# edouardoyallon/acco

Hardware: NVIDIA H100
Metric: tokens/sec (device-timed, max over ranks) Llama ACCO bf16 sharded-Adam, 8x1024 tokens per GPU per micro-batch (higher is better)
Workload: dtype bf16

## Files before the change

acco_b200/csrc/attention_wgmma.cu:

```cuda
#include <cuda.h>
#include <cuda_bf16.h>
#include <cuda_runtime.h>
#include <math.h>
#include <stdint.h>

#include "wgmma.cuh"

namespace acco_attn {

using namespace acco_tc;

constexpr int HD = 64;
constexpr int LDS = HD + 8;
constexpr float LOG2E = 1.4426950408889634f;
constexpr float LN2 = 0.6931471805599453f;

typedef __nv_bfloat16 bf16;

__device__ __forceinline__ uint32_t pack2(float a, float b) {
    __nv_bfloat162 h = __floats2bfloat162_rn(a, b);
    return *reinterpret_cast<uint32_t*>(&h);
}
__device__ __forceinline__ uint32_t ld32(const bf16* p) { return *reinterpret_cast<const uint32_t*>(p); }

__device__ __forceinline__ void mma16816(float (&c)[4], const uint32_t (&a)[4], uint32_t b0, uint32_t b1) {
    asm volatile("mma.sync.aligned.m16n8k16.row.col.f32.bf16.bf16.f32 {%0,%1,%2,%3}, {%4,%5,%6,%7}, {%8,%9}, {%0,%1,%2,%3};"
                 : "+f"(c[0]), "+f"(c[1]), "+f"(c[2]), "+f"(c[3])
                 : "r"(a[0]), "r"(a[1]), "r"(a[2]), "r"(a[3]), "r"(b0), "r"(b1));
}

template <int NB, int KB>
__device__ __forceinline__ void warp_mma_ss(float (&acc)[NB][4], const bf16* A, const bf16* B, int lane) {
    const int g = lane >> 2, t = lane & 3;
#pragma unroll
    for (int kb = 0; kb < KB; ++kb) {
        uint32_t a[4];
        const bf16* a0 = A + g * LDS + kb * 16 + 2 * t;
        a[0] = ld32(a0); a[1] = ld32(a0 + 8 * LDS); a[2] = ld32(a0 + 8); a[3] = ld32(a0 + 8 * LDS + 8);
#pragma unroll
        for (int nb = 0; nb < NB; ++nb) {
            const bf16* b = B + (nb * 8 + g) * LDS + kb * 16 + 2 * t;
            mma16816(acc[nb], a, ld32(b), ld32(b + 8));
        }
    }
}
template <int NB>
__device__ __forceinline__ void warp_mma_rs(float (&acc)[NB][4], const float (&p)[8][4], const bf16* B, int lane) {
    const int g = lane >> 2, t = lane & 3;
#pragma unroll
    for (int kb = 0; kb < 4; ++kb) {
        uint32_t a[4];
        a[0] = pack2(p[2 * kb][0], p[2 * kb][1]);
        a[1] = pack2(p[2 * kb][2], p[2 * kb][3]);
        a[2] = pack2(p[2 * kb + 1][0], p[2 * kb + 1][1]);
        a[3] = pack2(p[2 * kb + 1][2], p[2 * kb + 1][3]);
#pragma unroll
        for (int nb = 0; nb < NB; ++nb) {
            const bf16* b = B + (nb * 8 + g) * LDS + kb * 16 + 2 * t;
            mma16816(acc[nb], a, ld32(b), ld32(b + 8));
        }
    }
}

__device__ __forceinline__ void load_tile(bf16* dst, const bf16* src, long long ld, int rows, int valid, int tid, int nthr) {
    for (int i = tid; i < rows * 8; i += nthr) {
        const int r = i >> 3, c = (i & 7) * 8;
        uint4 v = make_uint4(0, 0, 0, 0);
        if (r < valid) v = *reinterpret_cast<const uint4*>(src + (long long)r * ld + c);
        *reinterpret_cast<uint4*>(dst + r * LDS + c) = v;
    }
}
__device__ __forceinline__ void load_tile_t(bf16* dst, const bf16* src, long long ld, int rows, int tid, int nthr) {
    for (int i = tid; i < rows * 8; i += nthr) {
        const int r = i >> 3, c = (i & 7) * 8;
        const uint4 v = *reinterpret_cast<const uint4*>(src + (long long)r * ld + c);
        const bf16* e = reinterpret_cast<const bf16*>(&v);
#pragma unroll
        for (int j = 0; j < 8; ++j) dst[(c + j) * LDS + r] = e[j];
    }
}

__device__ __forceinline__ bool visible(int q, int kv, int window) { return kv <= q && kv > q - window; }

struct FwdParams {
    CUtensorMap map_q;
    CUtensorMap map_k;
    CUtensorMap map_v;
    bf16* o;
    long long ld_o;
    float* lse;
    int B, S, Hq, Hk, window;
    float scale;
    const int* seg;
};

constexpr int FWD_Q = 128, FWD_KV = 64, FWD_THREADS = 256;
constexpr int FWD_TILE_KV = FWD_KV * HD * 2;
constexpr int FWD_SMEM = FWD_Q * HD * 2 + 2 * 2 * FWD_TILE_KV + 1024  + 64 ;

__device__ __forceinline__ void wgmma_m64n64k16_rs_tb(float (&d)[32], const uint32_t (&a)[4], uint64_t db) {
    asm volatile(
        "{\n\t.reg .pred p;\n\tsetp.ne.b32 p, %37, 0;\n\twgmma.mma_async.sync.aligned.m64n64k16.f32.bf16.bf16 "
        "{%0,%1,%2,%3,%4,%5,%6,%7,%8,%9,%10,%11,%12,%13,%14,%15,%16,%17,%18,%19,%20,%21,%22,%23,%24,%25,%26,%27,%28,%29,%30,%31}, "
        "{%32,%33,%34,%35}, %36, p, 1, 1, 1;\n\t}"
        : "+f"(d[0]), "+f"(d[1]), "+f"(d[2]), "+f"(d[3]), "+f"(d[4]), "+f"(d[5]), "+f"(d[6]), "+f"(d[7]), "+f"(d[8]), "+f"(d[9]), "+f"(d[10]),
          "+f"(d[11]), "+f"(d[12]), "+f"(d[13]), "+f"(d[14]), "+f"(d[15]), "+f"(d[16]), "+f"(d[17]), "+f"(d[18]), "+f"(d[19]), "+f"(d[20]),
          "+f"(d[21]), "+f"(d[22]), "+f"(d[23]), "+f"(d[24]), "+f"(d[25]), "+f"(d[26]), "+f"(d[27]), "+f"(d[28]), "+f"(d[29]), "+f"(d[30]),
          "+f"(d[31])
        : "r"(a[0]), "r"(a[1]), "r"(a[2]), "r"(a[3]), "l"(db), "r"(1));
}

template <bool kSeg>
__global__ void __launch_bounds__(FWD_THREADS) attn_fwd_kernel(const __grid_constant__ FwdParams P) {
    extern __shared__ uint8_t smem_raw[];
    uint8_t* smem = (uint8_t*)(((uintptr_t)smem_raw + 1023) & ~(uintptr_t)1023);
    uint8_t* sQ = smem;
    uint8_t* sKV = smem + FWD_Q * HD * 2;
    uint64_t* full = (uint64_t*)(sKV + 2 * 2 * FWD_TILE_KV);
    const int qb = blockIdx.x, h = blockIdx.y, b = blockIdx.z;
    const int hk = h / (P.Hq / P.Hk);
    const int tid = threadIdx.x, wg = tid >> 7, warp = (tid >> 5) & 3, lane = tid & 31, g = lane >> 2, t = lane & 3;
    const int q0 = qb * FWD_Q;
    const int row0 = b * P.S;
    int lo_key = max(0, q0 - P.window + 1);
    if constexpr (kSeg) lo_key = max(lo_key, P.seg[row0 + q0]);
    const int j_lo = lo_key / FWD_KV, j_hi = (q0 + FWD_Q - 1) / FWD_KV;
    auto issue = [&](int j) {
        const int s = (j - j_lo) & 1;
        mbar_expect_tx(&full[s], 2 * FWD_TILE_KV);
        tma_load_2d(&P.map_k, &full[s], sKV + s * 2 * FWD_TILE_KV, hk * HD, row0 + j * FWD_KV);
        tma_load_2d(&P.map_v, &full[s], sKV + s * 2 * FWD_TILE_KV + FWD_TILE_KV, hk * HD, row0 + j * FWD_KV);
    };
    if (tid == 0) {
        mbar_init(&full[0], 1);
        mbar_init(&full[1], 1);
        mbar_init(&full[2], 1);
        asm volatile("fence.mbarrier_init.release.cluster;" ::: "memory");
        mbar_expect_tx(&full[2], FWD_Q * HD * 2);
        tma_load_2d(&P.map_q, &full[2], sQ, h * HD, row0 + q0);
        issue(j_lo);
        if (j_lo + 1 <= j_hi) issue(j_lo + 1);
    }
    __syncthreads();
    mbar_wait(&full[2], 0);
    const float c = P.scale * LOG2E;
    float m_run[2] = {-INFINITY, -INFINITY}, l_run[2] = {0.f, 0.f};
    float o[32];
#pragma unroll
    for (int i = 0; i < 32; ++i) o[i] = 0.f;
    const int wq_lo = q0 + wg * 64, wq_hi = wq_lo + 63;
    const int qr[2] = {wq_lo + warp * 16 + g, wq_lo + warp * 16 + g + 8};
    int sg[2] = {0, 0}, wseg = 0;
    if constexpr (kSeg) {
        sg[0] = P.seg[row0 + qr[0]];
        sg[1] = P.seg[row0 + qr[1]];
        wseg = P.seg[row0 + wq_lo];
    }
    const uint32_t q_addr = smem_u32(sQ) + (uint32_t)(wg * 8192);
    for (int j = j_lo; j <= j_hi; ++j) {
        const int kv0 = j * FWD_KV, s = (j - j_lo) & 1;
        mbar_wait(&full[s], (uint32_t)(((j - j_lo) >> 1) & 1));
        if (!(kv0 > wq_hi || kv0 + FWD_KV - 1 <= wq_lo - P.window || (kSeg && kv0 + FWD_KV - 1 < wseg))) {
            const uint32_t k_addr = smem_u32(sKV + s * 2 * FWD_TILE_KV), v_addr = k_addr + FWD_TILE_KV;
            float sc[32];
#pragma unroll
            for (int i = 0; i < 32; ++i) sc[i] = 0.f;
            wgmma_fence();
#pragma unroll
            for (int k = 0; k < HD / 16; ++k)
                wgmma_m64n64k16<0, 0>(sc, make_smem_desc(q_addr + k * 32, 1, 1024 >> 4), make_smem_desc(k_addr + k * 32, 1, 1024 >> 4), 1u);
            wgmma_commit();
            wgmma_wait<0>();
            reg_fence(sc);
            float mx[2] = {-INFINITY, -INFINITY};
#pragma unroll
            for (int nb = 0; nb < 8; ++nb)
#pragma unroll
                for (int e = 0; e < 4; ++e) {
                    const int kv = kv0 + nb * 8 + 2 * t + (e & 1), r = e >> 1;
                    const float v = visible(qr[r], kv, P.window) && (!kSeg || kv >= sg[r]) ? sc[4 * nb + e] * c : -INFINITY;
                    sc[4 * nb + e] = v;
                    mx[r] = fmaxf(mx[r], v);
                }
#pragma unroll
            for (int r = 0; r < 2; ++r) {
                mx[r] = fmaxf(mx[r], __shfl_xor_sync(0xffffffffu, mx[r], 1));
                mx[r] = fmaxf(mx[r], __shfl_xor_sync(0xffffffffu, mx[r], 2));
            }
            float alpha[2], base[2], rs[2] = {0.f, 0.f};
#pragma unroll
            for (int r = 0; r < 2; ++r) {
                const float m_new = fmaxf(m_run[r], mx[r]);
                base[r] = m_new == -INFINITY ? 0.f : m_new;
                alpha[r] = exp2f(m_run[r] - base[r]);
                m_run[r] = m_new;
            }
#pragma unroll
            for (int i = 0; i < 32; ++i) {
                const int r = (i >> 1) & 1;
                const float p = exp2f(sc[i] - base[r]);
                sc[i] = p;
                rs[r] += p;
            }
#pragma unroll
            for (int r = 0; r < 2; ++r) {
                rs[r] += __shfl_xor_sync(0xffffffffu, rs[r], 1);
                rs[r] += __shfl_xor_sync(0xffffffffu, rs[r], 2);
                l_run[r] = l_run[r] * alpha[r] + rs[r];
            }
#pragma unroll
            for (int i = 0; i < 32; ++i) o[i] *= alpha[(i >> 1) & 1];
            wgmma_fence();
#pragma unroll
            for (int kk = 0; kk < FWD_KV / 16; ++kk) {
                uint32_t a[4];
                a[0] = pack2(sc[8 * kk + 0], sc[8 * kk + 1]);
                a[1] = pack2(sc[8 * kk + 2], sc[8 * kk + 3]);
                a[2] = pack2(sc[8 * kk + 4], sc[8 * kk + 5]);
                a[3] = pack2(sc[8 * kk + 6], sc[8 * kk + 7]);
                wgmma_m64n64k16_rs_tb(o, a, make_smem_desc(v_addr + kk * 2048, 8192 >> 4, 1024 >> 4));
            }
            wgmma_commit();
            wgmma_wait<0>();
            reg_fence(o);
        }
        __syncthreads();
        if (tid == 0 && j + 2 <= j_hi) issue(j + 2);
    }
#pragma unroll
    for (int r = 0; r < 2; ++r) {
        const int q = qr[r];
        const float inv = l_run[r] > 0.f ? 1.f / l_run[r] : 0.f;
        bf16* dst = P.o + ((long long)row0 + q) * P.ld_o + h * HD + 2 * t;
#pragma unroll
        for (int nb = 0; nb < 8; ++nb)
            *reinterpret_cast<uint32_t*>(dst + nb * 8) = pack2(o[4 * nb + 2 * r] * inv, o[4 * nb + 2 * r + 1] * inv);
        if (t == 0) P.lse[((long long)b * P.Hq + h) * P.S + q] = (m_run[r] + log2f(l_run[r])) * LN2;
    }
}

struct BwdParams {
    const bf16 *q, *k, *v;
    long long ld;
    const bf16* d_o;
    long long ld_do;
    const float *lse, *delta;
    float* dq;
    bf16 *dk, *dv;
    int B, S, Hq, Hk, window;
    float scale;
    const int* seg;
};

constexpr int BWD_KV = 64, BWD_Q = 64, BWD_THREADS = 128;
constexpr int BWD_SMEM = 8 * 64 * LDS * 2 + 2 * BWD_Q * 4;
constexpr int BWD_SMEM_SEG = BWD_SMEM + (BWD_Q + 1) * 4;

template <bool kSeg>
__global__ void __launch_bounds__(BWD_THREADS) attn_bwd_kernel(const BwdParams P) {
    extern __shared__ __align__(16) uint8_t smem_raw[];
    bf16* sK = reinterpret_cast<bf16*>(smem_raw);
    bf16* sKt = sK + 64 * LDS;
    bf16* sV = sKt + 64 * LDS;
    bf16* sQ = sV + 64 * LDS;
    bf16* sQt = sQ + 64 * LDS;
    bf16* sdO = sQt + 64 * LDS;
    bf16* sdOt = sdO + 64 * LDS;
    bf16* sdS = sdOt + 64 * LDS;
    float* sL = reinterpret_cast<float*>(sdS + 64 * LDS);
    float* sD = sL + BWD_Q;
    int* sSeg = reinterpret_cast<int*>(sD + BWD_Q);
    const int nb_k = blockIdx.x, hk = blockIdx.y, b = blockIdx.z;
    const int G = P.Hq / P.Hk;
    const int tid = threadIdx.x, warp = tid >> 5, lane = tid & 31, g = lane >> 2, t = lane & 3;
    const int kv0 = nb_k * BWD_KV;
    const long long row0 = (long long)b * P.S;
    load_tile(sK, P.k + (row0 + kv0) * P.ld + hk * HD, P.ld, BWD_KV, BWD_KV, tid, BWD_THREADS);
    load_tile_t(sKt, P.k + (row0 + kv0) * P.ld + hk * HD, P.ld, BWD_KV, tid, BWD_THREADS);
    load_tile(sV, P.v + (row0 + kv0) * P.ld + hk * HD, P.ld, BWD_KV, BWD_KV, tid, BWD_THREADS);
    const float c = P.scale * LOG2E;
    float dk[8][4], dv[8][4];
#pragma unroll
    for (int i = 0; i < 8; ++i)
#pragma unroll
        for (int e = 0; e < 4; ++e) dk[i][e] = dv[i][e] = 0.f;
    const int kr[2] = {kv0 + warp * 16 + g, kv0 + warp * 16 + g + 8};
    const int m_lo = kv0 / BWD_Q;
    const int m_hi = min(P.S / BWD_Q - 1, (kv0 + BWD_KV - 1 + P.window - 1) / BWD_Q);
    for (int gi = 0; gi < G; ++gi) {
        const int hq = hk * G + gi;
        for (int m = m_lo; m <= m_hi; ++m) {
            const int q0 = m * BWD_Q;
            __syncthreads();
            load_tile(sQ, P.q + (row0 + q0) * P.ld + hq * HD, P.ld, BWD_Q, BWD_Q, tid, BWD_THREADS);
            load_tile_t(sQt, P.q + (row0 + q0) * P.ld + hq * HD, P.ld, BWD_Q, tid, BWD_THREADS);
            load_tile(sdO, P.d_o + (row0 + q0) * P.ld_do + hq * HD, P.ld_do, BWD_Q, BWD_Q, tid, BWD_THREADS);
            load_tile_t(sdOt, P.d_o + (row0 + q0) * P.ld_do + hq * HD, P.ld_do, BWD_Q, tid, BWD_THREADS);
            if (tid < BWD_Q) {
                const long long li = ((long long)b * P.Hq + hq) * P.S + q0 + tid;
                sL[tid] = P.lse[li] * LOG2E;
                sD[tid] = P.delta[li];
                if constexpr (kSeg) sSeg[tid] = P.seg[row0 + q0 + tid];
            }
            if (kSeg && tid == BWD_Q) sSeg[BWD_Q] = m == m_hi || P.seg[row0 + q0 + BWD_Q] > kv0 + BWD_KV - 1;
            __syncthreads();
            float s[8][4], dp[8][4];
#pragma unroll
            for (int i = 0; i < 8; ++i)
#pragma unroll
                for (int e = 0; e < 4; ++e) s[i][e] = dp[i][e] = 0.f;
            warp_mma_ss<8, 4>(s, sK + warp * 16 * LDS, sQ, lane);
            warp_mma_ss<8, 4>(dp, sV + warp * 16 * LDS, sdO, lane);
#pragma unroll
            for (int nb = 0; nb < 8; ++nb)
#pragma unroll
                for (int e = 0; e < 4; ++e) {
                    const int ql = nb * 8 + 2 * t + (e & 1), q = q0 + ql, r = e >> 1;
                    const float p = visible(q, kr[r], P.window) && (!kSeg || kr[r] >= sSeg[ql]) ? exp2f(s[nb][e] * c - sL[ql]) : 0.f;
                    const float pb = __bfloat162float(__float2bfloat16(p));
                    s[nb][e] = pb;
                    dp[nb][e] = __bfloat162float(__float2bfloat16(p * (dp[nb][e] - sD[ql]) * P.scale));
                }
#pragma unroll
            for (int nb = 0; nb < 8; ++nb)
#pragma unroll
                for (int e = 0; e < 4; ++e) {
                    const int ql = nb * 8 + 2 * t + (e & 1), kl = warp * 16 + g + 8 * (e >> 1);
                    sdS[ql * LDS + kl] = __float2bfloat16(dp[nb][e]);
                }
            warp_mma_rs<8>(dv, s, sdOt, lane);
            warp_mma_rs<8>(dk, dp, sQt, lane);
            __syncthreads();
            float dq[8][4];
#pragma unroll
            for (int i = 0; i < 8; ++i) dq[i][0] = dq[i][1] = dq[i][2] = dq[i][3] = 0.f;
            warp_mma_ss<8, 4>(dq, sdS + warp * 16 * LDS, sKt, lane);
#pragma unroll
            for (int r = 0; r < 2; ++r) {
                float* dst = P.dq + (row0 + q0 + warp * 16 + g + 8 * r) * (long long)(P.Hq * HD) + hq * HD + 2 * t;
#pragma unroll
                for (int nb = 0; nb < 8; ++nb) {
                    atomicAdd(dst + nb * 8, dq[nb][2 * r]);
                    atomicAdd(dst + nb * 8 + 1, dq[nb][2 * r + 1]);
                }
            }
            if (kSeg && sSeg[BWD_Q]) break;
        }
    }
#pragma unroll
    for (int r = 0; r < 2; ++r) {
        const long long off = (row0 + kr[r]) * (long long)(P.Hk * HD) + hk * HD + 2 * t;
#pragma unroll
        for (int nb = 0; nb < 8; ++nb) {
            *reinterpret_cast<uint32_t*>(P.dk + off + nb * 8) = pack2(dk[nb][2 * r], dk[nb][2 * r + 1]);
            *reinterpret_cast<uint32_t*>(P.dv + off + nb * 8) = pack2(dv[nb][2 * r], dv[nb][2 * r + 1]);
        }
    }
}

__global__ void __launch_bounds__(256) attn_delta_kernel(const bf16* __restrict__ o, const bf16* __restrict__ d_o, long long ld_o,
                                                         long long ld_do, float* __restrict__ delta, int B, int S, int Hq) {
    const long long item = ((long long)blockIdx.x * blockDim.x + threadIdx.x) >> 3;
    const int part = threadIdx.x & 7;
    const long long n_items = (long long)B * S * Hq;
    float acc = 0.f;
    long long row = 0;
    int h = 0;
    if (item < n_items) {
        row = item / Hq;
        h = (int)(item - row * Hq);
        const uint4 a = *reinterpret_cast<const uint4*>(o + row * ld_o + h * HD + part * 8);
        const uint4 d = *reinterpret_cast<const uint4*>(d_o + row * ld_do + h * HD + part * 8);
        const __nv_bfloat162* a2 = reinterpret_cast<const __nv_bfloat162*>(&a);
        const __nv_bfloat162* d2 = reinterpret_cast<const __nv_bfloat162*>(&d);
#pragma unroll
        for (int i = 0; i < 4; ++i) {
            const float2 x = __bfloat1622float2(a2[i]), y = __bfloat1622float2(d2[i]);
            acc += x.x * y.x + x.y * y.y;
        }
    }
    acc += __shfl_xor_sync(0xffffffffu, acc, 1);
    acc += __shfl_xor_sync(0xffffffffu, acc, 2);
    acc += __shfl_xor_sync(0xffffffffu, acc, 4);
    if (item < n_items && part == 0) {
        const long long b = row / S, s = row - b * S;
        delta[(b * Hq + h) * S + s] = acc;
    }
}

static bool shape_ok(int B, int S, int Hq, int Hk, int D, float scale) {
    return B > 0 && S > 0 && S % 128 == 0 && Hk > 0 && Hq > 0 && Hq % Hk == 0 && D == HD && scale > 0.f;
}
static bool aligned(const void* p, long long ld) { return ((uintptr_t)p % 16) == 0 && (ld % 8) == 0; }
static int eff_window(int S, int window) { return (window <= 0 || window > S) ? S : window; }

}

extern "C" int acco_attn_supported(int B, int S, int Hq, int Hk, int D, float scale) {
    return acco_attn::shape_ok(B, S, Hq, Hk, D, scale) ? 1 : 0;
}

extern "C" int acco_attn_fwd(const void* q, const void* k, const void* v, long long ld, void* o, long long ld_o, float* lse, int B, int S, int Hq,
                             int Hk, int D, float scale, int window, const int* seg, cudaStream_t st) {
    using namespace acco_attn;
    if (!shape_ok(B, S, Hq, Hk, D, scale) || !aligned(q, ld) || !aligned(k, ld) || !aligned(v, ld) || !aligned(o, ld_o)) return -1;
    static int fwd_attr = (int)cudaFuncSetAttribute(attn_fwd_kernel<false>, cudaFuncAttributeMaxDynamicSharedMemorySize, FWD_SMEM);
    static int fwd_attr_seg = (int)cudaFuncSetAttribute(attn_fwd_kernel<true>, cudaFuncAttributeMaxDynamicSharedMemorySize, FWD_SMEM);
    if (fwd_attr) return fwd_attr;
    if (fwd_attr_seg) return fwd_attr_seg;
    FwdParams P;
    const uint64_t rows = (uint64_t)B * S;
    int rc = acco_gemm::make_map_typed(&P.map_q, q, (uint64_t)Hq * HD, rows, (uint64_t)ld, HD, FWD_Q, 2);
    if (!rc) rc = acco_gemm::make_map_typed(&P.map_k, k, (uint64_t)Hk * HD, rows, (uint64_t)ld, HD, FWD_KV, 2);
    if (!rc) rc = acco_gemm::make_map_typed(&P.map_v, v, (uint64_t)Hk * HD, rows, (uint64_t)ld, HD, FWD_KV, 2);
    if (rc) return rc;
    P.o = (bf16*)o; P.ld_o = ld_o; P.lse = lse;
    P.B = B; P.S = S; P.Hq = Hq; P.Hk = Hk; P.window = eff_window(S, window); P.scale = scale; P.seg = seg;
    if (seg)
        attn_fwd_kernel<true><<<dim3(S / FWD_Q, Hq, B), FWD_THREADS, FWD_SMEM, st>>>(P);
    else
        attn_fwd_kernel<false><<<dim3(S / FWD_Q, Hq, B), FWD_THREADS, FWD_SMEM, st>>>(P);
    return (int)cudaGetLastError();
}

extern "C" int acco_attn_bwd(const void* q, const void* k, const void* v, long long ld, const void* o, long long ld_o, const void* d_o,
                             long long ld_do, const float* lse, float* delta, float* dq_acc, void* dk, void* dv, int B, int S, int Hq, int Hk, int D,
                             float scale, int window, const int* seg, cudaStream_t st) {
    using namespace acco_attn;
    if (!shape_ok(B, S, Hq, Hk, D, scale) || !aligned(q, ld) || !aligned(k, ld) || !aligned(v, ld) || !aligned(o, ld_o) || !aligned(d_o, ld_do))
        return -1;
    static int attr_rc = (int)cudaFuncSetAttribute(attn_bwd_kernel<false>, cudaFuncAttributeMaxDynamicSharedMemorySize, BWD_SMEM);
    static int attr_rc_seg = (int)cudaFuncSetAttribute(attn_bwd_kernel<true>, cudaFuncAttributeMaxDynamicSharedMemorySize, BWD_SMEM_SEG);
    if (attr_rc) return attr_rc;
    if (attr_rc_seg) return attr_rc_seg;
    const long long items = (long long)B * S * Hq;
    attn_delta_kernel<<<(unsigned)((items * 8 + 255) / 256), 256, 0, st>>>((const bf16*)o, (const bf16*)d_o, ld_o, ld_do, delta, B, S, Hq);
    if (cudaMemsetAsync(dq_acc, 0, (size_t)items * HD * sizeof(float), st) != cudaSuccess) return -6;
    BwdParams P{(const bf16*)q, (const bf16*)k, (const bf16*)v, ld, (const bf16*)d_o, ld_do, lse, delta, dq_acc, (bf16*)dk, (bf16*)dv,
                B, S, Hq, Hk, eff_window(S, window), scale, seg};
    if (seg)
        attn_bwd_kernel<true><<<dim3(S / BWD_KV, Hk, B), BWD_THREADS, BWD_SMEM_SEG, st>>>(P);
    else
        attn_bwd_kernel<false><<<dim3(S / BWD_KV, Hk, B), BWD_THREADS, BWD_SMEM, st>>>(P);
    return (int)cudaGetLastError();
}
```

Measured before the change: 387,100.

## Rewrite attention backward with WGMMA, TMA double-buffering and TMA reduce for dQ

The attention backward kernel moves from warp-level mma.sync with manually transposed shared-memory tiles to Hopper WGMMA. It now uses two warpgroups over a 128-key block, TMA loads of Q/dO/LSE/delta double-buffered with mbarriers, and TMA reduce-add of dQ through a swizzled shared buffer in place of per-element atomics. This is meant to remove the scalar transpose loads, the redundant smem copies and the heavy global atomic traffic. The forward grid is reordered so heads come first and query blocks run in reverse order, putting the long causal blocks early. The cost is a large, complex kernel with new alignment requirements on lse/delta/seg and one block per SM.

```diff
diff --git a/acco_b200/csrc/attention_wgmma.cu b/acco_b200/csrc/attention_wgmma.cu
--- a/acco_b200/csrc/attention_wgmma.cu
+++ b/acco_b200/csrc/attention_wgmma.cu
@@ -11,7 +11,6 @@
 using namespace acco_tc;
 
 constexpr int HD = 64;
-constexpr int LDS = HD + 8;
 constexpr float LOG2E = 1.4426950408889634f;
 constexpr float LN2 = 0.6931471805599453f;
 
@@ -20,64 +19,6 @@
 __device__ __forceinline__ uint32_t pack2(float a, float b) {
     __nv_bfloat162 h = __floats2bfloat162_rn(a, b);
     return *reinterpret_cast<uint32_t*>(&h);
-}
-__device__ __forceinline__ uint32_t ld32(const bf16* p) { return *reinterpret_cast<const uint32_t*>(p); }
-
-__device__ __forceinline__ void mma16816(float (&c)[4], const uint32_t (&a)[4], uint32_t b0, uint32_t b1) {
-    asm volatile("mma.sync.aligned.m16n8k16.row.col.f32.bf16.bf16.f32 {%0,%1,%2,%3}, {%4,%5,%6,%7}, {%8,%9}, {%0,%1,%2,%3};"
-                 : "+f"(c[0]), "+f"(c[1]), "+f"(c[2]), "+f"(c[3])
-                 : "r"(a[0]), "r"(a[1]), "r"(a[2]), "r"(a[3]), "r"(b0), "r"(b1));
-}
-
-template <int NB, int KB>
-__device__ __forceinline__ void warp_mma_ss(float (&acc)[NB][4], const bf16* A, const bf16* B, int lane) {
-    const int g = lane >> 2, t = lane & 3;
-#pragma unroll
-    for (int kb = 0; kb < KB; ++kb) {
-        uint32_t a[4];
-        const bf16* a0 = A + g * LDS + kb * 16 + 2 * t;
-        a[0] = ld32(a0); a[1] = ld32(a0 + 8 * LDS); a[2] = ld32(a0 + 8); a[3] = ld32(a0 + 8 * LDS + 8);
-#pragma unroll
-        for (int nb = 0; nb < NB; ++nb) {
-            const bf16* b = B + (nb * 8 + g) * LDS + kb * 16 + 2 * t;
-            mma16816(acc[nb], a, ld32(b), ld32(b + 8));
-        }
-    }
-}
-template <int NB>
-__device__ __forceinline__ void warp_mma_rs(float (&acc)[NB][4], const float (&p)[8][4], const bf16* B, int lane) {
-    const int g = lane >> 2, t = lane & 3;
-#pragma unroll
-    for (int kb = 0; kb < 4; ++kb) {
-        uint32_t a[4];
-        a[0] = pack2(p[2 * kb][0], p[2 * kb][1]);
-        a[1] = pack2(p[2 * kb][2], p[2 * kb][3]);
-        a[2] = pack2(p[2 * kb + 1][0], p[2 * kb + 1][1]);
-        a[3] = pack2(p[2 * kb + 1][2], p[2 * kb + 1][3]);
-#pragma unroll
-        for (int nb = 0; nb < NB; ++nb) {
-            const bf16* b = B + (nb * 8 + g) * LDS + kb * 16 + 2 * t;
-            mma16816(acc[nb], a, ld32(b), ld32(b + 8));
-        }
-    }
-}
-
-__device__ __forceinline__ void load_tile(bf16* dst, const bf16* src, long long ld, int rows, int valid, int tid, int nthr) {
-    for (int i = tid; i < rows * 8; i += nthr) {
-        const int r = i >> 3, c = (i & 7) * 8;
-        uint4 v = make_uint4(0, 0, 0, 0);
-        if (r < valid) v = *reinterpret_cast<const uint4*>(src + (long long)r * ld + c);
-        *reinterpret_cast<uint4*>(dst + r * LDS + c) = v;
-    }
-}
-__device__ __forceinline__ void load_tile_t(bf16* dst, const bf16* src, long long ld, int rows, int tid, int nthr) {
-    for (int i = tid; i < rows * 8; i += nthr) {
-        const int r = i >> 3, c = (i & 7) * 8;
-        const uint4 v = *reinterpret_cast<const uint4*>(src + (long long)r * ld + c);
-        const bf16* e = reinterpret_cast<const bf16*>(&v);
-#pragma unroll
-        for (int j = 0; j < 8; ++j) dst[(c + j) * LDS + r] = e[j];
-    }
 }
 
 __device__ __forceinline__ bool visible(int q, int kv, int window) { return kv <= q && kv > q - window; }
@@ -117,9 +58,10 @@
     uint8_t* sQ = smem;
     uint8_t* sKV = smem + FWD_Q * HD * 2;
     uint64_t* full = (uint64_t*)(sKV + 2 * 2 * FWD_TILE_KV);
-    const int qb = blockIdx.x, h = blockIdx.y, b = blockIdx.z;
+    const int h = blockIdx.x, b = blockIdx.y, qb = gridDim.z - 1 - blockIdx.z;
     const int hk = h / (P.Hq / P.Hk);
-    const int tid = threadIdx.x, wg = tid >> 7, warp = (tid >> 5) & 3, lane = tid & 31, g = lane >> 2, t = lane & 3;
+    const int tid = threadIdx.x, warp = (tid >> 5) & 3, lane = tid & 31, g = lane >> 2, t = lane & 3;
+    const int wg = __shfl_sync(0xffffffffu, tid >> 7, 0);
     const int q0 = qb * FWD_Q;
     const int row0 = b * P.S;
     int lo_key = max(0, q0 - P.window + 1);
@@ -240,120 +182,188 @@
 }
 
 struct BwdParams {
-    const bf16 *q, *k, *v;
-    long long ld;
-    const bf16* d_o;
-    long long ld_do;
+    CUtensorMap map_q;
+    CUtensorMap map_k;
+    CUtensorMap map_v;
+    CUtensorMap map_do;
+    CUtensorMap map_dq;
     const float *lse, *delta;
-    float* dq;
     bf16 *dk, *dv;
     int B, S, Hq, Hk, window;
     float scale;
     const int* seg;
 };
 
-constexpr int BWD_KV = 64, BWD_Q = 64, BWD_THREADS = 128;
-constexpr int BWD_SMEM = 8 * 64 * LDS * 2 + 2 * BWD_Q * 4;
-constexpr int BWD_SMEM_SEG = BWD_SMEM + (BWD_Q + 1) * 4;
+constexpr int BWD_KV = 128, BWD_Q = 64, BWD_THREADS = 256;
+constexpr int BWD_TILE = BWD_Q * HD * 2;
+constexpr int BWD_STAGE = 2 * BWD_TILE + 3 * BWD_Q * 4;
+constexpr int BWD_DQ = BWD_Q * HD * 4;
+constexpr int BWD_SMEM = 2 * 2 * BWD_TILE + 2 * BWD_TILE + 2 * BWD_DQ + 2 * BWD_STAGE + 1024  + 64 ;
+
+__device__ __forceinline__ void bulk_load(void* dst, const void* src, uint32_t bytes, uint64_t* bar) {
+    asm volatile("cp.async.bulk.shared::cluster.global.mbarrier::complete_tx::bytes [%0], [%1], %2, [%3];" ::"r"(smem_u32(dst)), "l"(src),
+                 "r"(bytes), "r"(smem_u32(bar))
+                 : "memory");
+}
 
 template <bool kSeg>
-__global__ void __launch_bounds__(BWD_THREADS) attn_bwd_kernel(const BwdParams P) {
-    extern __shared__ __align__(16) uint8_t smem_raw[];
-    bf16* sK = reinterpret_cast<bf16*>(smem_raw);
-    bf16* sKt = sK + 64 * LDS;
-    bf16* sV = sKt + 64 * LDS;
-    bf16* sQ = sV + 64 * LDS;
-    bf16* sQt = sQ + 64 * LDS;
-    bf16* sdO = sQt + 64 * LDS;
-    bf16* sdOt = sdO + 64 * LDS;
-    bf16* sdS = sdOt + 64 * LDS;
-    float* sL = reinterpret_cast<float*>(sdS + 64 * LDS);
-    float* sD = sL + BWD_Q;
-    int* sSeg = reinterpret_cast<int*>(sD + BWD_Q);
-    const int nb_k = blockIdx.x, hk = blockIdx.y, b = blockIdx.z;
+__global__ void __launch_bounds__(BWD_THREADS, 1) attn_bwd_kernel(const __grid_constant__ BwdParams P) {
+    extern __shared__ uint8_t smem_raw[];
+    uint8_t* smem = (uint8_t*)(((uintptr_t)smem_raw + 1023) & ~(uintptr_t)1023);
+    uint8_t* sK = smem;
+    uint8_t* sV = sK + 2 * BWD_TILE;
+    uint8_t* sDS = sV + 2 * BWD_TILE;
+    uint8_t* sDQ = sDS + 2 * BWD_TILE;
+    uint8_t* sStage = sDQ + 2 * BWD_DQ;
+    uint64_t* full = (uint64_t*)(sStage + 2 * BWD_STAGE);
+    const int hk = blockIdx.x, b = blockIdx.y, n = blockIdx.z;
     const int G = P.Hq / P.Hk;
-    const int tid = threadIdx.x, warp = tid >> 5, lane = tid & 31, g = lane >> 2, t = lane & 3;
-    const int kv0 = nb_k * BWD_KV;
-    const long long row0 = (long long)b * P.S;
-    load_tile(sK, P.k + (row0 + kv0) * P.ld + hk * HD, P.ld, BWD_KV, BWD_KV, tid, BWD_THREADS);
-    load_tile_t(sKt, P.k + (row0 + kv0) * P.ld + hk * HD, P.ld, BWD_KV, tid, BWD_THREADS);
-    load_tile(sV, P.v + (row0 + kv0) * P.ld + hk * HD, P.ld, BWD_KV, BWD_KV, tid, BWD_THREADS);
-    const float c = P.scale * LOG2E;
-    float dk[8][4], dv[8][4];
-#pragma unroll
-    for (int i = 0; i < 8; ++i)
-#pragma unroll
-        for (int e = 0; e < 4; ++e) dk[i][e] = dv[i][e] = 0.f;
-    const int kr[2] = {kv0 + warp * 16 + g, kv0 + warp * 16 + g + 8};
+    const int tid = threadIdx.x, warp = (tid >> 5) & 3, lane = tid & 31, g = lane >> 2, t = lane & 3;
+    const int wg = __shfl_sync(0xffffffffu, tid >> 7, 0);
+    const int kv0 = n * BWD_KV;
+    const int row0 = b * P.S;
     const int m_lo = kv0 / BWD_Q;
     const int m_hi = min(P.S / BWD_Q - 1, (kv0 + BWD_KV - 1 + P.window - 1) / BWD_Q);
-    for (int gi = 0; gi < G; ++gi) {
-        const int hq = hk * G + gi;
-        for (int m = m_lo; m <= m_hi; ++m) {
-            const int q0 = m * BWD_Q;
-            __syncthreads();
-            load_tile(sQ, P.q + (row0 + q0) * P.ld + hq * HD, P.ld, BWD_Q, BWD_Q, tid, BWD_THREADS);
-            load_tile_t(sQt, P.q + (row0 + q0) * P.ld + hq * HD, P.ld, BWD_Q, tid, BWD_THREADS);
-            load_tile(sdO, P.d_o + (row0 + q0) * P.ld_do + hq * HD, P.ld_do, BWD_Q, BWD_Q, tid, BWD_THREADS);
-            load_tile_t(sdOt, P.d_o + (row0 + q0) * P.ld_do + hq * HD, P.ld_do, BWD_Q, tid, BWD_THREADS);
-            if (tid < BWD_Q) {
-                const long long li = ((long long)b * P.Hq + hq) * P.S + q0 + tid;
-                sL[tid] = P.lse[li] * LOG2E;
-                sD[tid] = P.delta[li];
-                if constexpr (kSeg) sSeg[tid] = P.seg[row0 + q0 + tid];
-            }
-            if (kSeg && tid == BWD_Q) sSeg[BWD_Q] = m == m_hi || P.seg[row0 + q0 + BWD_Q] > kv0 + BWD_KV - 1;
-            __syncthreads();
-            float s[8][4], dp[8][4];
-#pragma unroll
-            for (int i = 0; i < 8; ++i)
-#pragma unroll
-                for (int e = 0; e < 4; ++e) s[i][e] = dp[i][e] = 0.f;
-            warp_mma_ss<8, 4>(s, sK + warp * 16 * LDS, sQ, lane);
-            warp_mma_ss<8, 4>(dp, sV + warp * 16 * LDS, sdO, lane);
+    int m_end = m_hi + 1;
+    if constexpr (kSeg) {
+        m_end = m_lo + 1;
+        while (m_end <= m_hi && P.seg[row0 + m_end * BWD_Q] <= kv0 + BWD_KV - 1) ++m_end;
+    }
+    const int nm = m_end - m_lo, n_items = G * nm;
+    auto stage = [&](int s) { return sStage + s * BWD_STAGE; };
+    auto issue = [&](int it) {
+        const int s = it & 1, hq = hk * G + it / nm, q0 = (m_lo + it % nm) * BWD_Q;
+        uint8_t* st = stage(s);
+        const long long li = ((long long)b * P.Hq + hq) * P.S + q0;
+        mbar_expect_tx(&full[s], 2 * BWD_TILE + (kSeg ? 3 : 2) * BWD_Q * 4);
+        tma_load_2d(&P.map_q, &full[s], st, hq * HD, row0 + q0);
+        tma_load_2d(&P.map_do, &full[s], st + BWD_TILE, hq * HD, row0 + q0);
+        bulk_load(st + 2 * BWD_TILE, P.lse + li, BWD_Q * 4, &full[s]);
+        bulk_load(st + 2 * BWD_TILE + BWD_Q * 4, P.delta + li, BWD_Q * 4, &full[s]);
+        if constexpr (kSeg) bulk_load(st + 2 * BWD_TILE + 2 * BWD_Q * 4, P.seg + row0 + q0, BWD_Q * 4, &full[s]);
+    };
+    if (tid == 0) {
+        mbar_init(&full[0], 1);
+        mbar_init(&full[1], 1);
+        mbar_init(&full[2], 1);
+        asm volatile("fence.mbarrier_init.release.cluster;" ::: "memory");
+        mbar_expect_tx(&full[2], 2 * 2 * BWD_TILE);
+        tma_load_2d(&P.map_k, &full[2], sK, hk * HD, row0 + kv0);
+        tma_load_2d(&P.map_v, &full[2], sV, hk * HD, row0 + kv0);
+        issue(0);
+        if (n_items > 1) issue(1);
+    }
+    __syncthreads();
+    mbar_wait(&full[2], 0);
+    const float c = P.scale * LOG2E;
+    float dk[32], dv[32];
+#pragma unroll
+    for (int i = 0; i < 32; ++i) dk[i] = dv[i] = 0.f;
+    const int wk_lo = kv0 + wg * 64, wk_hi = wk_lo + 63;
+    const int kr[2] = {wk_lo + warp * 16 + g, wk_lo + warp * 16 + g + 8};
+    const uint32_t k_addr = smem_u32(sK) + (uint32_t)(wg * BWD_TILE), v_addr = smem_u32(sV) + (uint32_t)(wg * BWD_TILE);
+    uint8_t* ds = sDS + wg * BWD_TILE;
+    for (int it = 0; it < n_items; ++it) {
+        const int s = it & 1, hq = hk * G + it / nm, q0 = (m_lo + it % nm) * BWD_Q;
+        const uint8_t* st = stage(s);
+        const float* sL = reinterpret_cast<const float*>(st + 2 * BWD_TILE);
+        const float* sD = sL + BWD_Q;
+        const int* sSeg = reinterpret_cast<const int*>(sD + BWD_Q);
+        mbar_wait(&full[s], (uint32_t)((it >> 1) & 1));
+        if (!(wk_lo > q0 + BWD_Q - 1 || wk_hi <= q0 - P.window || (kSeg && sSeg[0] > wk_hi))) {
+            const uint32_t q_addr = smem_u32(st), do_addr = q_addr + BWD_TILE;
+            float sc[32], dp[32];
+#pragma unroll
+            for (int i = 0; i < 32; ++i) sc[i] = dp[i] = 0.f;
+            wgmma_fence();
+#pragma unroll
+            for (int k = 0; k < HD / 16; ++k)
+                wgmma_m64n64k16<0, 0>(sc, make_smem_desc(k_addr + k * 32, 1, 1024 >> 4), make_smem_desc(q_addr + k * 32, 1, 1024 >> 4), 1u);
+#pragma unroll
+            for (int k = 0; k < HD / 16; ++k)
+                wgmma_m64n64k16<0, 0>(dp, make_smem_desc(v_addr + k * 32, 1, 1024 >> 4), make_smem_desc(do_addr + k * 32, 1, 1024 >> 4), 1u);
+            wgmma_commit();
+            wgmma_wait<0>();
+            reg_fence(sc);
+            reg_fence(dp);
 #pragma unroll
             for (int nb = 0; nb < 8; ++nb)
 #pragma unroll
                 for (int e = 0; e < 4; ++e) {
-                    const int ql = nb * 8 + 2 * t + (e & 1), q = q0 + ql, r = e >> 1;
-                    const float p = visible(q, kr[r], P.window) && (!kSeg || kr[r] >= sSeg[ql]) ? exp2f(s[nb][e] * c - sL[ql]) : 0.f;
-                    const float pb = __bfloat162float(__float2bfloat16(p));
-                    s[nb][e] = pb;
-                    dp[nb][e] = __bfloat162float(__float2bfloat16(p * (dp[nb][e] - sD[ql]) * P.scale));
+                    const int i = 4 * nb + e, ql = nb * 8 + 2 * t + (e & 1), r = e >> 1;
+                    const bool vis = visible(q0 + ql, kr[r], P.window) && (!kSeg || kr[r] >= sSeg[ql]);
+                    const float p = vis ? exp2f(sc[i] * c - sL[ql] * LOG2E) : 0.f;
+                    sc[i] = __bfloat162float(__float2bfloat16(p));
+                    dp[i] = __bfloat162float(__float2bfloat16(p * (dp[i] - sD[ql]) * P.scale));
                 }
 #pragma unroll
             for (int nb = 0; nb < 8; ++nb)
 #pragma unroll
-                for (int e = 0; e < 4; ++e) {
-                    const int ql = nb * 8 + 2 * t + (e & 1), kl = warp * 16 + g + 8 * (e >> 1);
-                    sdS[ql * LDS + kl] = __float2bfloat16(dp[nb][e]);
-                }
-            warp_mma_rs<8>(dv, s, sdOt, lane);
-            warp_mma_rs<8>(dk, dp, sQt, lane);
-            __syncthreads();
-            float dq[8][4];
-#pragma unroll
-            for (int i = 0; i < 8; ++i) dq[i][0] = dq[i][1] = dq[i][2] = dq[i][3] = 0.f;
-            warp_mma_ss<8, 4>(dq, sdS + warp * 16 * LDS, sKt, lane);
-#pragma unroll
-            for (int r = 0; r < 2; ++r) {
-                float* dst = P.dq + (row0 + q0 + warp * 16 + g + 8 * r) * (long long)(P.Hq * HD) + hq * HD + 2 * t;
-#pragma unroll
-                for (int nb = 0; nb < 8; ++nb) {
-                    atomicAdd(dst + nb * 8, dq[nb][2 * r]);
-                    atomicAdd(dst + nb * 8 + 1, dq[nb][2 * r + 1]);
-                }
-            }
-            if (kSeg && sSeg[BWD_Q]) break;
+                for (int r = 0; r < 2; ++r)
+                    *reinterpret_cast<uint32_t*>(ds + (warp * 16 + g + 8 * r) * 128 + ((nb ^ g) << 4) + 4 * t) =
+                        pack2(dp[4 * nb + 2 * r], dp[4 * nb + 2 * r + 1]);
+            fence_async_smem();
+            if ((tid & 127) == 0) bulk_wait_read<0>();
+            named_barrier(1 + wg, 128);
+            float dq[32];
+#pragma unroll
+            for (int i = 0; i < 32; ++i) dq[i] = 0.f;
+            wgmma_fence();
+#pragma unroll
+            for (int kk = 0; kk < BWD_Q / 16; ++kk) {
+                uint32_t a[4];
+                a[0] = pack2(sc[8 * kk + 0], sc[8 * kk + 1]);
+                a[1] = pack2(sc[8 * kk + 2], sc[8 * kk + 3]);
+                a[2] = pack2(sc[8 * kk + 4], sc[8 * kk + 5]);
+                a[3] = pack2(sc[8 * kk + 6], sc[8 * kk + 7]);
+                wgmma_m64n64k16_rs_tb(dv, a, make_smem_desc(do_addr + kk * 2048, BWD_TILE >> 4, 1024 >> 4));
+            }
+#pragma unroll
+            for (int kk = 0; kk < BWD_Q / 16; ++kk) {
+                uint32_t a[4];
+                a[0] = pack2(dp[8 * kk + 0], dp[8 * kk + 1]);
+                a[1] = pack2(dp[8 * kk + 2], dp[8 * kk + 3]);
+                a[2] = pack2(dp[8 * kk + 4], dp[8 * kk + 5]);
+                a[3] = pack2(dp[8 * kk + 6], dp[8 * kk + 7]);
+                wgmma_m64n64k16_rs_tb(dk, a, make_smem_desc(q_addr + kk * 2048, BWD_TILE >> 4, 1024 >> 4));
+            }
+            const uint32_t ds_addr = smem_u32(ds);
+#pragma unroll
+            for (int kk = 0; kk < 64 / 16; ++kk)
+                wgmma_m64n64k16<1, 1>(dq, make_smem_desc(ds_addr + kk * 2048, BWD_TILE >> 4, 1024 >> 4),
+                                      make_smem_desc(k_addr + kk * 2048, BWD_TILE >> 4, 1024 >> 4), 1u);
+            wgmma_commit();
+            wgmma_wait<0>();
+            reg_fence(dv);
+            reg_fence(dk);
+            reg_fence(dq);
+            uint8_t* dqs = sDQ + wg * BWD_DQ;
+#pragma unroll
+            for (int nb = 0; nb < 8; ++nb)
+#pragma unroll
+                for (int r = 0; r < 2; ++r)
+                    *reinterpret_cast<float2*>(dqs + (nb >> 2) * (BWD_DQ / 2) + (warp * 16 + g + 8 * r) * 128 +
+                                               (((((nb & 3) << 1) | (t >> 1)) ^ g) << 4) + (t & 1) * 8) =
+                        make_float2(dq[4 * nb + 2 * r], dq[4 * nb + 2 * r + 1]);
+            fence_async_smem();
+            named_barrier(1 + wg, 128);
+            if ((tid & 127) == 0) {
+                tma_reduce_add_2d(&P.map_dq, dqs, hq * HD, row0 + q0);
+                tma_reduce_add_2d(&P.map_dq, dqs + BWD_DQ / 2, hq * HD + 32, row0 + q0);
+                bulk_commit();
+            }
         }
-    }
+        __syncthreads();
+        if (tid == 0 && it + 2 < n_items) issue(it + 2);
+    }
+    if ((tid & 127) == 0) bulk_wait<0>();
 #pragma unroll
     for (int r = 0; r < 2; ++r) {
-        const long long off = (row0 + kr[r]) * (long long)(P.Hk * HD) + hk * HD + 2 * t;
+        const long long off = ((long long)row0 + kr[r]) * (long long)(P.Hk * HD) + hk * HD + 2 * t;
 #pragma unroll
         for (int nb = 0; nb < 8; ++nb) {
-            *reinterpret_cast<uint32_t*>(P.dk + off + nb * 8) = pack2(dk[nb][2 * r], dk[nb][2 * r + 1]);
-            *reinterpret_cast<uint32_t*>(P.dv + off + nb * 8) = pack2(dv[nb][2 * r], dv[nb][2 * r + 1]);
+            *reinterpret_cast<uint32_t*>(P.dk + off + nb * 8) = pack2(dk[4 * nb + 2 * r], dk[4 * nb + 2 * r + 1]);
+            *reinterpret_cast<uint32_t*>(P.dv + off + nb * 8) = pack2(dv[4 * nb + 2 * r], dv[4 * nb + 2 * r + 1]);
         }
     }
 }
@@ -417,9 +427,9 @@
     P.o = (bf16*)o; P.ld_o = ld_o; P.lse = lse;
     P.B = B; P.S = S; P.Hq = Hq; P.Hk = Hk; P.window = eff_window(S, window); P.scale = scale; P.seg = seg;
     if (seg)
-        attn_fwd_kernel<true><<<dim3(S / FWD_Q, Hq, B), FWD_THREADS, FWD_SMEM, st>>>(P);
+        attn_fwd_kernel<true><<<dim3(Hq, B, S / FWD_Q), FWD_THREADS, FWD_SMEM, st>>>(P);
     else
-        attn_fwd_kernel<false><<<dim3(S / FWD_Q, Hq, B), FWD_THREADS, FWD_SMEM, st>>>(P);
+        attn_fwd_kernel<false><<<dim3(Hq, B, S / FWD_Q), FWD_THREADS, FWD_SMEM, st>>>(P);
     return (int)cudaGetLastError();
 }
 
@@ -429,18 +439,28 @@
     using namespace acco_attn;
     if (!shape_ok(B, S, Hq, Hk, D, scale) || !aligned(q, ld) || !aligned(k, ld) || !aligned(v, ld) || !aligned(o, ld_o) || !aligned(d_o, ld_do))
         return -1;
+    if ((uintptr_t)lse % 16 || (uintptr_t)delta % 16 || (seg && (uintptr_t)seg % 16)) return -1;
     static int attr_rc = (int)cudaFuncSetAttribute(attn_bwd_kernel<false>, cudaFuncAttributeMaxDynamicSharedMemorySize, BWD_SMEM);
-    static int attr_rc_seg = (int)cudaFuncSetAttribute(attn_bwd_kernel<true>, cudaFuncAttributeMaxDynamicSharedMemorySize, BWD_SMEM_SEG);
+    static int attr_rc_seg = (int)cudaFuncSetAttribute(attn_bwd_kernel<true>, cudaFuncAttributeMaxDynamicSharedMemorySize, BWD_SMEM);
     if (attr_rc) return attr_rc;
     if (attr_rc_seg) return attr_rc_seg;
+    BwdParams P;
+    const uint64_t rows = (uint64_t)B * S;
+    int rc = acco_gemm::make_map_typed(&P.map_q, q, (uint64_t)Hq * HD, rows, (uint64_t)ld, HD, BWD_Q, 2);
+    if (!rc) rc = acco_gemm::make_map_typed(&P.map_k, k, (uint64_t)Hk * HD, rows, (uint64_t)ld, HD, BWD_KV, 2);
+    if (!rc) rc = acco_gemm::make_map_typed(&P.map_v, v, (uint64_t)Hk * HD, rows, (uint64_t)ld, HD, BWD_KV, 2);
+    if (!rc) rc = acco_gemm::make_map_typed(&P.map_do, d_o, (uint64_t)Hq * HD, rows, (uint64_t)ld_do, HD, BWD_Q, 2);
+    if (!rc) rc = acco_gemm::make_map_typed(&P.map_dq, dq_acc, (uint64_t)Hq * HD, rows, (uint64_t)Hq * HD, 32, BWD_Q, 4);
+    if (rc) return rc;
     const long long items = (long long)B * S * Hq;
     attn_delta_kernel<<<(unsigned)((items * 8 + 255) / 256), 256, 0, st>>>((const bf16*)o, (const bf16*)d_o, ld_o, ld_do, delta, B, S, Hq);
     if (cudaMemsetAsync(dq_acc, 0, (size_t)items * HD * sizeof(float), st) != cudaSuccess) return -6;
-    BwdParams P{(const bf16*)q, (const bf16*)k, (const bf16*)v, ld, (const bf16*)d_o, ld_do, lse, delta, dq_acc, (bf16*)dk, (bf16*)dv,
-                B, S, Hq, Hk, eff_window(S, window), scale, seg};
+    P.lse = lse; P.delta = delta; P.dk = (bf16*)dk; P.dv = (bf16*)dv;
+    P.B = B; P.S = S; P.Hq = Hq; P.Hk = Hk; P.window = eff_window(S, window); P.scale = scale; P.seg = seg;
+    const dim3 grid(Hk, B, S / BWD_KV);
     if (seg)
-        attn_bwd_kernel<true><<<dim3(S / BWD_KV, Hk, B), BWD_THREADS, BWD_SMEM_SEG, st>>>(P);
+        attn_bwd_kernel<true><<<grid, BWD_THREADS, BWD_SMEM, st>>>(P);
     else
-        attn_bwd_kernel<false><<<dim3(S / BWD_KV, Hk, B), BWD_THREADS, BWD_SMEM, st>>>(P);
+        attn_bwd_kernel<false><<<grid, BWD_THREADS, BWD_SMEM, st>>>(P);
     return (int)cudaGetLastError();
 }
```

New measurement: 387,200, median of 6. No clear change (+0.0%).
